# Fabri000/Maze-Solving-Agent-Gymnasium

Hardware: NVIDIA B200
Metric: env-steps/sec (40x40 mazes, whole job) (higher is better)
Workload: dtype u8/int32 state+obs, f64 reward

## Files before the change

### maze-solving-agent-gymnasium_b200/csrc/maze_abi.cu

```cuda
#include <cmath>
#include <cstdio>
#include <cstdlib>
#include <cstring>
#include <new>
#include "maze_common.cuh"

int maze_fail_cuda(maze_ctx* ctx, cudaError_t e, const char* what) {
    if (ctx) snprintf(ctx->err, sizeof(ctx->err), "CUDA error %d (%s) in %s", (int)e, cudaGetErrorString(e), what);
    return (int)e;
}

int maze_fail_arg(maze_ctx* ctx, int code, const char* what) {
    if (ctx) snprintf(ctx->err, sizeof(ctx->err), "argument error %d: %s", code, what);
    return code;
}

int maze_check_batch(maze_ctx* ctx, const maze_env_batch* b) {
    if (!b) return maze_fail_arg(ctx, MAZE_E_NULL, "batch");
    if (!b->meta || !b->table || !b->env_maze || !b->state || !b->visits || !b->agent || !b->target ||
        !b->best_dir || !b->reward || !b->terminated || !b->truncated)
        return maze_fail_arg(ctx, MAZE_E_NULL, "batch pointer");
    if (b->num_envs <= 0 || b->num_mazes <= 0 || b->slot <= 0 || (b->slot & 1))
        return maze_fail_arg(ctx, MAZE_E_RANGE, "num_envs / num_mazes / slot (must be even)");
    if (b->visit_slot < b->slot || (b->visit_tiled != 0 && b->visit_tiled != 1))
        return maze_fail_arg(ctx, MAZE_E_RANGE, "visit_slot (>= slot) / visit_tiled (0 or 1)");
    if (b->visit_bits && (b->visit_bits_pitch < 1 || b->visit_bits_stride < b->visit_bits_pitch || (b->visit_bits_stride & 3) ||
                          ((uintptr_t)b->visit_bits & 15)))
        return maze_fail_arg(ctx, MAZE_E_RANGE, "visit_bits: pitch >= 1, stride a multiple of 4 words, 16-byte aligned");
    if (b->visit_cell_stride <= 0 || b->visit_env_stride <= 0)
        return maze_fail_arg(ctx, MAZE_E_RANGE, "visit strides (cell-major: B, 1; env-major: 1, slot)");
    if (((uintptr_t)b->meta & 15) || ((uintptr_t)b->state & 7) || ((uintptr_t)b->agent & 7) ||
        ((uintptr_t)b->target & 7) || ((uintptr_t)b->best_dir & 7) || ((uintptr_t)b->reward & 7) ||
        ((uintptr_t)b->visits & 3))
        return maze_fail_arg(ctx, MAZE_E_ALIGN, "batch pointer alignment");
    return 0;
}


extern "C" int maze_abi_version(void) { return MAZE_ABI_VERSION; }

extern "C" int maze_sizeof(int which) {
    switch (which) {
        case 0: return (int)sizeof(maze_env_batch);
        case 1: return (int)sizeof(maze_q_agent);
        case 2: return (int)sizeof(maze_replay);
        case 3: return (int)sizeof(maze_step_trace);
        case 4: return (int)sizeof(maze_dqn_net);
        default: return -1;
    }
}

extern "C" int maze_ctx_create(maze_ctx** out, int device) {
    if (!out) return MAZE_E_NULL;
    *out = nullptr;
    maze_ctx* ctx = new (std::nothrow) maze_ctx();
    if (!ctx) return MAZE_E_RANGE;
    memset(ctx, 0, sizeof(*ctx));
    ctx->device = device;
    for (int i = 0; i < 256; ++i) {
        ctx->h_lut_revisit[i] = 0.0 - (1 - std::exp(-0.2 * i));
        ctx->h_lut_invalid[i] = 0.0 - (1 - std::exp(-0.15 * i));
    }
    ctx->h_shaping[0] = 0 * 0.5 - 0.05;
    ctx->h_shaping[1] = 1 * 0.5 - 0.05;
    ctx->h_shaping[2] = 0.0;
    ctx->h_shaping[3] = -1 * 0.5 - 0.05;
    cudaError_t e = cudaSetDevice(device);
    if (e == cudaSuccess) e = cudaMalloc(&ctx->d_lut_revisit, 256 * sizeof(double));
    if (e == cudaSuccess) e = cudaMalloc(&ctx->d_lut_invalid, 256 * sizeof(double));
    if (e == cudaSuccess) e = cudaMalloc(&ctx->d_counter, 4 * sizeof(int));
    if (e == cudaSuccess) e = cudaMemcpy(ctx->d_lut_revisit, ctx->h_lut_revisit, 256 * sizeof(double), cudaMemcpyHostToDevice);
    if (e == cudaSuccess) e = cudaMemcpy(ctx->d_lut_invalid, ctx->h_lut_invalid, 256 * sizeof(double), cudaMemcpyHostToDevice);
    if (e == cudaSuccess) e = cudaDeviceGetAttribute(&ctx->num_sms, cudaDevAttrMultiProcessorCount, device);
    if (e != cudaSuccess) {
        int rc = (int)e;
        cudaFree(ctx->d_lut_revisit);
        cudaFree(ctx->d_lut_invalid);
        cudaFree(ctx->d_counter);
        delete ctx;
        return rc;
    }
    ctx->step_ept = 2;
    if (const char* v = getenv("MAZE_STEP_EPT")) ctx->step_ept = atoi(v);
    if (const char* v = getenv("MAZE_L2_PERSIST_MB")) {
        int maxp = 0;
        cudaDeviceGetAttribute(&maxp, cudaDevAttrMaxPersistingL2CacheSize, device);
        size_t want = (size_t)atoi(v) << 20, before = 0, after = 0;
        if (want > (size_t)maxp) want = (size_t)maxp;
        cudaDeviceGetLimit(&before, cudaLimitPersistingL2CacheSize);
        cudaError_t le = cudaDeviceSetLimit(cudaLimitPersistingL2CacheSize, want);
        cudaDeviceGetLimit(&after, cudaLimitPersistingL2CacheSize);
        fprintf(stderr, "[maze_b200] persisting L2 %zu -> %zu bytes (max %d, rc %d)\n", before, after, maxp, (int)le);
    }
    if (const char* v = getenv("MAZE_L2_FETCH")) {
        size_t before = 0, after = 0;
        cudaDeviceGetLimit(&before, cudaLimitMaxL2FetchGranularity);
        cudaError_t le = cudaDeviceSetLimit(cudaLimitMaxL2FetchGranularity, (size_t)atoi(v));
        cudaDeviceGetLimit(&after, cudaLimitMaxL2FetchGranularity);
        fprintf(stderr, "[maze_b200] L2 fetch granularity %zu -> %zu (rc %d)\n", before, after, (int)le);
    }
    *out = ctx;
    return 0;
}

extern "C" void maze_ctx_destroy(maze_ctx* ctx) {
    if (!ctx) return;
    cudaFree(ctx->d_lut_revisit);
    cudaFree(ctx->d_lut_invalid);
    cudaFree(ctx->d_counter);
    cudaFree(ctx->d_scratch);
    maze_net_profile_free(ctx);
    delete ctx;
}

extern "C" const char* maze_last_error(maze_ctx* ctx) { return ctx ? ctx->err : "null ctx"; }

extern "C" int maze_reward_lut(maze_ctx* ctx, int kind, double* out) {
    if (!out) return MAZE_E_NULL;
    double rev[256], inv[256];
    for (int i = 0; i < 256; ++i) {
        rev[i] = 0.0 - (1 - std::exp(-0.2 * i));
        inv[i] = 0.0 - (1 - std::exp(-0.15 * i));
    }
    memset(out, 0, 256 * sizeof(double));
    if (kind == 0) memcpy(out, rev, sizeof(rev));
    else if (kind == 1) memcpy(out, inv, sizeof(inv));
    else if (kind == 2) { out[0] = -1 * 0.5 - 0.05; out[1] = 0 * 0.5 - 0.05; out[2] = 1 * 0.5 - 0.05; }
    else return maze_fail_arg(ctx, MAZE_E_RANGE, "maze_reward_lut kind");
    return 0;
}

extern "C" int maze_step_decode_host(const uint32_t* records, int64_t n, const int32_t* shape, const uint8_t* toroidal, int32_t* agent,
                                     int32_t* best_dir, double* reward, uint8_t* terminated, uint8_t* truncated) {
    if (!records || n < 0) return MAZE_E_NULL;
    double lut[4][256];
    memset(lut, 0, sizeof(lut));
    for (int i = 0; i < 256; ++i) {
        lut[MAZE_REC_KIND_REVISIT][i] = 0.0 - (1 - std::exp(-0.2 * i));
        lut[MAZE_REC_KIND_INVALID][i] = 0.0 - (1 - std::exp(-0.15 * i));
    }
    lut[MAZE_REC_KIND_SHAPING][0] = -1 * 0.5 - 0.05;
    lut[MAZE_REC_KIND_SHAPING][1] = 0 * 0.5 - 0.05;
    lut[MAZE_REC_KIND_SHAPING][2] = 1 * 0.5 - 0.05;
    lut[MAZE_REC_KIND_CONST][MAZE_REC_CONST_ONE] = 1.0;
    lut[MAZE_REC_KIND_CONST][MAZE_REC_CONST_MINUS_ONE] = -1.0;
    for (int64_t e = 0; e < n; ++e) {
        const uint32_t rec = records[e];
        const int r = (int)(rec & 0xff), c = (int)((rec >> 8) & 0xff), code = (int)((rec >> MAZE_REC_CODE_SHIFT) & 7);
        if (agent) { agent[2 * e] = r; agent[2 * e + 1] = c; }
        if (best_dir) {
            int br = 0, bc = 0;
            if (code < 4) {
                const int dr = (code == 0) - (code == 1), dc = (code == 2) - (code == 3);
                int nr = r + dr, nc = c + dc;
                if (toroidal && toroidal[e] && shape) {
                    const int H = shape[2 * e], W = shape[2 * e + 1];
                    nr = nr < 0 ? H - 1 : (nr >= H ? 0 : nr);
                    nc = nc < 0 ? W - 1 : (nc >= W ? 0 : nc);
                }
                br = r - nr;
                bc = c - nc;
            }
            best_dir[2 * e] = br;
            best_dir[2 * e + 1] = bc;
        }
        if (reward) reward[e] = lut[(rec >> MAZE_REC_KIND_SHIFT) & 3][(rec >> MAZE_REC_INDEX_SHIFT) & 0xff];
        if (terminated) terminated[e] = (uint8_t)((rec >> MAZE_REC_TERM_SHIFT) & 1);
        if (truncated) truncated[e] = (uint8_t)((rec >> MAZE_REC_TRUNC_SHIFT) & 1);
    }
    return 0;
}
```

### maze-solving-agent-gymnasium_b200/csrc/maze_common.cuh

```cuda
#pragma once
#include <cuda_runtime.h>
#include <stdint.h>
#include "maze_b200.h"

#define MAZE_CHECK(call)                                                          \
    do {                                                                          \
        cudaError_t _e = (call);                                                  \
        if (_e != cudaSuccess) return maze_fail_cuda(ctx, _e, #call);             \
    } while (0)

struct maze_ctx {
    int device;
    double* d_lut_revisit;
    double* d_lut_invalid;
    int*    d_counter;
    double h_lut_revisit[256];
    double h_lut_invalid[256];
    double h_shaping[4];
    int    num_sms;
    int    step_ept;
    void*  d_scratch;
    size_t scratch_bytes;
    void*  net_profile;
    char   err[512];
};

void maze_net_profile_free(maze_ctx* ctx);
int maze_fail_cuda(maze_ctx* ctx, cudaError_t e, const char* what);
int maze_fail_arg(maze_ctx* ctx, int code, const char* what);
int maze_check_batch(maze_ctx* ctx, const maze_env_batch* b);

struct EnvState {
    int r, c, consec, flags, steps, epoch, tab;
};

__device__ __forceinline__ EnvState unpack_state(uint64_t s) {
    EnvState e;
    e.r = (int)(s & 0xff);
    e.c = (int)((s >> 8) & 0xff);
    e.consec = (int)((s >> 16) & 0xff);
    e.flags = (int)((s >> 24) & 0xff);
    e.steps = (int)((s >> 32) & 0xffff);
    e.epoch = (int)((s >> 48) & 0xff);
    e.tab = (int)((s >> 56) & 0xff);
    return e;
}

__device__ __forceinline__ uint64_t pack_state(const EnvState& e) {
    uint32_t lo = (uint32_t)e.r | ((uint32_t)e.c << 8) | ((uint32_t)e.consec << 16) | ((uint32_t)e.flags << 24);
    uint32_t hi = (uint32_t)e.steps | ((uint32_t)e.epoch << 16) | ((uint32_t)e.tab << 24);
    return (uint64_t)lo | ((uint64_t)hi << 32);
}

__device__ __forceinline__ void action_delta(int a, int& dr, int& dc) {
    dr = (a == 0) - (a == 1);
    dc = (a == 2) - (a == 3);
}

__device__ __forceinline__ int2 best_dir_from_code(int code, int r, int c, int H, int W, bool tor) {
    if (code >= 4) return make_int2(0, 0);
    int dr, dc;
    action_delta(code, dr, dc);
    int nr = r + dr, nc = c + dc;
    if (tor) {
        nr = nr < 0 ? H - 1 : (nr >= H ? 0 : nr);
        nc = nc < 0 ? W - 1 : (nc >= W ? 0 : nc);
    }
    return make_int2(r - nr, c - nc);
}

__device__ __forceinline__ void st_cs(int2* p, int2 v) { __stcs(p, v); }
__device__ __forceinline__ void st_cs(double* p, double v) { __stcs(p, v); }

struct Philox {
    uint32_t k0, k1;
    uint32_t c0, c1, c2, c3;
    uint32_t o0, o1, o2, o3;
    int have;

    __host__ __device__ void init(uint64_t seed, uint64_t seq, uint32_t sub = 0) {
        k0 = (uint32_t)seed;
        k1 = (uint32_t)(seed >> 32);
        c0 = 0; c1 = sub;
        c2 = (uint32_t)seq;
        c3 = (uint32_t)(seq >> 32);
        have = 0;
    }
    __host__ __device__ static inline void mulhilo(uint32_t a, uint32_t b, uint32_t& hi, uint32_t& lo) {
        uint64_t p = (uint64_t)a * b;
        hi = (uint32_t)(p >> 32);
        lo = (uint32_t)p;
    }
    __host__ __device__ void refill() {
        uint32_t x0 = c0, x1 = c1, x2 = c2, x3 = c3, a = k0, b = k1;
#pragma unroll
        for (int i = 0; i < 10; ++i) {
            uint32_t hi0, lo0, hi1, lo1;
            mulhilo(0xD2511F53u, x0, hi0, lo0);
            mulhilo(0xCD9E8D57u, x2, hi1, lo1);
            uint32_t y0 = hi1 ^ x1 ^ a, y1 = lo1, y2 = hi0 ^ x3 ^ b, y3 = lo0;
            x0 = y0; x1 = y1; x2 = y2; x3 = y3;
            a += 0x9E3779B9u; b += 0xBB67AE85u;
        }
        o0 = x0; o1 = x1; o2 = x2; o3 = x3;
        if (++c0 == 0) ++c1;
        have = 4;
    }
    __host__ __device__ uint32_t next() {
        if (have == 0) refill();
        const uint32_t v = o0;
        o0 = o1; o1 = o2; o2 = o3;
        --have;
        return v;
    }
    __host__ __device__ uint32_t below(uint32_t n) {
        return (uint32_t)(((uint64_t)next() * n) >> 32);
    }
};
```

### maze-solving-agent-gymnasium_b200/csrc/maze_step.cu

```cuda
#include "maze_env.cuh"

namespace {

constexpr int STEP_THREADS = 256;
#ifndef MAZE_STEP_MINB1
#define MAZE_STEP_MINB1 6
#endif
#ifndef MAZE_STEP_MINB4
#define MAZE_STEP_MINB4 2
#endif
#ifndef MAZE_STEP_MINB2
#define MAZE_STEP_MINB2 5
#endif

template <int EPT, bool kStats, bool kTiled>
__global__ void __launch_bounds__(STEP_THREADS, EPT == 2 ? MAZE_STEP_MINB2 : (EPT == 1 ? MAZE_STEP_MINB1 : MAZE_STEP_MINB4))
maze_step_kernel(maze_env_batch b, const uint8_t* __restrict__ actions, uint32_t mode, StepLuts luts) {
    const int base = blockIdx.x * (STEP_THREADS * EPT) + threadIdx.x;

    const uint64_t pol_state = l2_policy<MAZE_STATE_POLICY>(), pol_table = l2_policy<MAZE_TABLE_POLICY>();
    uint64_t raw[EPT];
    int m[EPT], a[EPT];
    bool valid[EPT];
#pragma unroll
    for (int k = 0; k < EPT; ++k) {
        const int e = base + k * STEP_THREADS;
        valid[k] = e < b.num_envs;
        const int ee = valid[k] ? e : b.num_envs - 1;
        raw[k] = pol_load<MAZE_STATE_POLICY>(reinterpret_cast<const unsigned long long*>(b.state) + ee, pol_state);
        m[k] = pol_load<MAZE_STATE_POLICY>(b.env_maze + ee, pol_state);
        a[k] = __ldcs(actions + ee) & 3;
    }

    bool do_reset[EPT];
    int hw[EPT], tor[EPT];
#pragma unroll
    for (int k = 0; k < EPT; ++k) {
        const int flags = (int)((raw[k] >> 24) & 0xff);
        do_reset[k] = valid[k] && (mode & MAZE_STEP_AUTORESET) && (flags & MAZE_ST_NEEDS_RESET);
        if (do_reset[k] && (mode & MAZE_STEP_WIN_NEXT) && (flags & MAZE_ST_WON)) {
            m[k] += b.pool_stride;
            if (m[k] >= b.num_mazes) m[k] -= b.num_mazes;
            pol_store<MAZE_STATE_POLICY>(b.env_maze + base + k * STEP_THREADS, m[k], pol_state);
        }
        const int2 shape = __ldg(reinterpret_cast<const int2*>(b.meta + (size_t)m[k] * MAZE_META_WORDS));
        hw[k] = shape.x | (shape.y << 16);
        tor[k] = __ldg(b.meta + (size_t)m[k] * MAZE_META_WORDS + MAZE_META_FLAGS) & MAZE_FLAG_TOROIDAL;
    }

    int npos[EPT], idx[EPT], vidx[EPT], tb[EPT];
    bool inb[EPT];
#pragma unroll
    for (int k = 0; k < EPT; ++k) {
        const int H = hw[k] & 0xffff, W = hw[k] >> 16;
        const int r = (int)(raw[k] & 0xff), c = (int)((raw[k] >> 8) & 0xff);
        int dr, dc;
        action_delta(a[k], dr, dc);
        int nr = r + dr, nc = c + dc;
        if (tor[k]) {
            nr = nr < 0 ? H - 1 : (nr >= H ? 0 : nr);
            nc = nc < 0 ? W - 1 : (nc >= W ? 0 : nc);
            inb[k] = true;
        } else {
            inb[k] = (nr > 0) & (nr < H - 1) & (nc > 0) & (nc < W - 1);
        }
        if (do_reset[k]) {
            const int start = __ldg(b.meta + (size_t)m[k] * MAZE_META_WORDS + MAZE_META_START);
            nr = start & 0xffff;
            nc = start >> 16;
            inb[k] = true;
        }
        if (!inb[k]) { nr = r; nc = c; }
        npos[k] = nr | (nc << 16);
        idx[k] = nr * W + nc;
        vidx[k] = kTiled ? ((((nr >> 2) * ((W + 3) >> 2) + (nc >> 2)) << 4) | ((nr & 3) << 2) | (nc & 3)) : idx[k];
#ifdef MAZE_EXP_NOTABLE
        tb[k] = 1 | ((idx[k] & 3) << 1) | ((idx[k] & 3) << 4);
#else
        tb[k] = pol_load_nc<MAZE_TABLE_POLICY>(b.table + (size_t)m[k] * b.slot + idx[k], pol_table);
#endif
    }

    const uint64_t pol = l2_policy<MAZE_VISIT_POLICY>();
    uint32_t vis[EPT];
    bool moved[EPT];
#pragma unroll
    for (int k = 0; k < EPT; ++k) {
        moved[k] = valid[k] && !do_reset[k] && inb[k] && (tb[k] & MAZE_TAB_OPEN);
        vis[k] = 0;
#ifndef MAZE_EXP_NOVISIT
        if (moved[k]) vis[k] = visit_load(VISIT_AT(b, base + k * STEP_THREADS, vidx[k]), pol);
#endif
    }

#pragma unroll
    for (int k = 0; k < EPT; ++k) {
        const int e = base + k * STEP_THREADS;
        const int H = hw[k] & 0xffff, W = hw[k] >> 16;
        const int goal = __ldg(b.meta + (size_t)m[k] * MAZE_META_WORDS + MAZE_META_GOAL);
        const int max_steps = __ldg(b.meta + (size_t)m[k] * MAZE_META_WORDS + MAZE_META_MAX_STEPS);
        double reward = 0.0;
        int term = 0, trunc = 0;
        uint32_t rcode = MAZE_REC_REWARD(MAZE_REC_KIND_CONST, MAZE_REC_CONST_ZERO);
        bool wrapped = false;
        EnvState st = unpack_state(raw[k]);

        if (do_reset[k]) {
            begin_episode(st, npos[k], tb[k], wrapped);
            visit_bits_clear(b, e);
        } else if (valid[k]) {
            if (moved[k]) {
                const int cnt = ((int)(vis[k] >> 8) == st.epoch) ? (int)(vis[k] & 0xff) : 0;
                if (cnt == 0) {
                    if (npos[k] == goal) {
                        reward = 1.0;
                        term = 1;
                        rcode = MAZE_REC_REWARD(MAZE_REC_KIND_CONST, MAZE_REC_CONST_ONE);
                    } else {
                        const int dd = ((st.tab >> MAZE_TAB_D4_SHIFT) - (tb[k] >> MAZE_TAB_D4_SHIFT)) & 3;
                        reward = dd == 1 ? luts.shaping_closer : (dd == 3 ? luts.shaping_farther : luts.shaping_same);
                        rcode = MAZE_REC_REWARD(MAZE_REC_KIND_SHAPING, dd == 1 ? 2u : (dd == 3 ? 0u : 1u));
                    }
                } else {
                    reward = __ldg(luts.revisit + cnt);
                    rcode = MAZE_REC_REWARD(MAZE_REC_KIND_REVISIT, (uint32_t)cnt);
                }
#ifndef MAZE_EXP_NOVISIT
                visit_store(VISIT_AT(b, e, vidx[k]), (unsigned)((st.epoch << 8) | (cnt < 255 ? cnt + 1 : 255)), pol);
                visit_bit_set(b, e, npos[k] & 0xffff, npos[k] >> 16);
#endif
                st.r = npos[k] & 0xffff;
                st.c = npos[k] >> 16;
                st.tab = tb[k];
                st.consec = 0;
                int nm = (st.flags >> MAZE_ST_NMOVES_SHIFT) & 3;
                nm = nm < 2 ? nm + 1 : 2;
                st.flags = (a[k] << MAZE_ST_MOVE_SHIFT) | (nm << MAZE_ST_NMOVES_SHIFT);
            } else {
                st.consec = st.consec < 255 ? st.consec + 1 : 255;
                reward = __ldg(luts.invalid + st.consec);
                rcode = MAZE_REC_REWARD(MAZE_REC_KIND_INVALID, (uint32_t)st.consec);
                st.flags &= ~(MAZE_ST_NEEDS_RESET | MAZE_ST_WON);
            }
            st.steps = st.steps < 65535 ? st.steps + 1 : 65535;
            if (st.steps > max_steps) {
                trunc = 1;
                reward = -1.0;
                rcode = MAZE_REC_REWARD(MAZE_REC_KIND_CONST, MAZE_REC_CONST_MINUS_ONE);
            }
            if (term | trunc) st.flags |= MAZE_ST_NEEDS_RESET | (term ? MAZE_ST_WON : 0);
        }

        const unsigned need = __ballot_sync(0xffffffffu, wrapped);
        if (need) warp_clear_visits(need, b, e);
        if (kStats && b.stats) {
            const unsigned stepped = __ballot_sync(0xffffffffu, valid[k] && !do_reset[k]);
            if (stepped && (threadIdx.x & 31) == 0) atomicAdd(reinterpret_cast<unsigned long long*>(b.stats + 3), (unsigned long long)__popc(stepped));
        }

        if (!valid[k]) continue;

        pol_store<MAZE_STATE_POLICY>(reinterpret_cast<unsigned long long*>(b.state) + e, (unsigned long long)pack_state(st), pol_state);
        if (do_reset[k] && (raw[k] >> 24 & MAZE_ST_WON)) {
            st_cs(reinterpret_cast<int2*>(b.target) + e, make_int2(goal & 0xffff, goal >> 16));
            if (b.target_dirty) *b.target_dirty = 1;
        }
        if (mode & MAZE_STEP_PACKED)
            __stcs(b.packed + e, (uint32_t)st.r | ((uint32_t)st.c << 8) | ((uint32_t)((st.tab >> MAZE_TAB_CODE_SHIFT) & 7) << MAZE_REC_CODE_SHIFT) |
                                     ((uint32_t)term << MAZE_REC_TERM_SHIFT) | ((uint32_t)trunc << MAZE_REC_TRUNC_SHIFT) | rcode);
        if (!(mode & MAZE_STEP_NO_WIDE)) {
            st_cs(reinterpret_cast<int2*>(b.agent) + e, make_int2(st.r, st.c));
            st_cs(reinterpret_cast<int2*>(b.best_dir) + e,
                  best_dir_from_code((st.tab >> MAZE_TAB_CODE_SHIFT) & 7, st.r, st.c, H, W, tor[k] != 0));
            st_cs(b.reward + e, reward);
            __stcs(b.terminated + e, (uint8_t)term);
            __stcs(b.truncated + e, (uint8_t)trunc);
        }

        if (kStats) {
            if (b.ep_return) {
                double g = do_reset[k] ? 0.0 : b.ep_return[e] + reward;
                b.ep_return[e] = g;
                if ((term | trunc) && b.stats_return) atomicAdd(b.stats_return, g);
            }
            if (b.stats) {
                if (term | trunc) {
                    atomicAdd(reinterpret_cast<unsigned long long*>(b.stats + 0), 1ull);
                    if (term) atomicAdd(reinterpret_cast<unsigned long long*>(b.stats + 1), 1ull);
                    else atomicAdd(reinterpret_cast<unsigned long long*>(b.stats + 2), 1ull);
                }
            }
            if (term && (mode & MAZE_STEP_WIN_QUEUE) && b.queue) {
                int at = atomicAdd(b.queue_count, 1);
                b.queue[at] = m[k];
            }
        }
    }
}

__global__ void __launch_bounds__(STEP_THREADS)
maze_reset_kernel(maze_env_batch b, const uint8_t* __restrict__ mask) {
    const int e = blockIdx.x * STEP_THREADS + threadIdx.x;
    const bool valid = e < b.num_envs;
    const int ee = valid ? e : b.num_envs - 1;
    const bool sel = valid && (mask == nullptr || mask[ee] != 0);
    bool wrapped = false;
    EnvState s;
    int H = 0, W = 0, goal = 0;
    bool tor = false;
    if (sel) {
        s = unpack_state(b.state[ee]);
        const int m = b.env_maze[ee];
        const int4* mp = reinterpret_cast<const int4*>(b.meta + (size_t)m * MAZE_META_WORDS);
        const int4 m0 = __ldg(mp);
        const int4 m1 = __ldg(mp + 1);
        H = m0.x; W = m0.y; goal = m0.w;
        tor = (m1.y & MAZE_FLAG_TOROIDAL) != 0;
        const int start = m0.z;
        const int sidx = (start & 0xffff) * W + (start >> 16);
        begin_episode(s, start, __ldg(b.table + (size_t)m * b.slot + sidx), wrapped);
        visit_bits_clear(b, ee);
    }
    const unsigned need = __ballot_sync(0xffffffffu, wrapped);
    if (need) warp_clear_visits(need, b, ee);
    if (!sel) return;
    b.state[e] = pack_state(s);
    reinterpret_cast<int2*>(b.agent)[e] = make_int2(s.r, s.c);
    reinterpret_cast<int2*>(b.target)[e] = make_int2(goal & 0xffff, goal >> 16);
    if (b.target_dirty) *b.target_dirty = 1;
    reinterpret_cast<int2*>(b.best_dir)[e] =
        best_dir_from_code((s.tab >> MAZE_TAB_CODE_SHIFT) & 7, s.r, s.c, H, W, tor);
    b.reward[e] = 0.0;
    b.terminated[e] = 0;
    b.truncated[e] = 0;
    if (b.ep_return) b.ep_return[e] = 0.0;
}

__global__ void __launch_bounds__(STEP_THREADS)
maze_step_many_kernel(maze_env_batch b, const uint8_t* __restrict__ actions, int k_steps, uint32_t mode, StepLuts luts,
                      maze_step_trace tr, int e0, int e1) {
    const int e = e0 + blockIdx.x * STEP_THREADS + threadIdx.x;
    if (e >= e1) return;
    const size_t B = (size_t)b.num_envs;
    EnvState st = unpack_state(b.state[e]);
    int m = b.env_maze[e];
    MazeView mz = load_maze(b, m);
    double reward = 0.0, ep_return = b.ep_return ? b.ep_return[e] : 0.0;
    int term = 0, trunc = 0;
    bool target_changed = false;
    unsigned long long n_episodes = 0, n_wins = 0, n_steps = 0;
    double return_sum = 0.0;
    for (int k = 0; k < k_steps; ++k) {
        if ((mode & MAZE_STEP_AUTORESET) && (st.flags & MAZE_ST_NEEDS_RESET)) {
            if ((mode & MAZE_STEP_WIN_NEXT) && (st.flags & MAZE_ST_WON)) {
                m += b.pool_stride;
                if (m >= b.num_mazes) m -= b.num_mazes;
                mz = load_maze(b, m);
            }
            bool wrapped;
            begin_episode(st, mz.start, __ldg(mz.tab + (mz.start & 0xffff) * mz.W + (mz.start >> 16)), wrapped);
            visit_bits_clear(b, e);
            if (wrapped)
                for (int i = 0; i < b.visit_slot; ++i) *VISIT_AT(b, e, i) = 0;
            reward = 0.0; term = 0; trunc = 0;
            ep_return = 0.0;
            target_changed = true;
        } else {
            const StepResult r = env_transition(b, e, st, mz, __ldcs(actions + (size_t)k * B + e) & 3, luts);
            reward = r.reward; term = r.term; trunc = r.trunc;
            ep_return += reward;
            ++n_steps;
            if (term | trunc) {
                ++n_episodes;
                n_wins += term;
                return_sum += ep_return;
            }
        }
        const size_t at = (size_t)k * B + e;
        if (tr.agent) __stcs(reinterpret_cast<int2*>(tr.agent) + at, make_int2(st.r, st.c));
        if (tr.best_dir)
            __stcs(reinterpret_cast<int2*>(tr.best_dir) + at,
                   best_dir_from_code((st.tab >> MAZE_TAB_CODE_SHIFT) & 7, st.r, st.c, mz.H, mz.W, mz.tor));
        if (tr.reward) __stcs(tr.reward + at, reward);
        if (tr.terminated) __stcs(tr.terminated + at, (uint8_t)term);
        if (tr.truncated) __stcs(tr.truncated + at, (uint8_t)trunc);
    }
    b.state[e] = pack_state(st);
    b.env_maze[e] = m;
    reinterpret_cast<int2*>(b.agent)[e] = make_int2(st.r, st.c);
    if (target_changed) {
        reinterpret_cast<int2*>(b.target)[e] = make_int2(mz.goal & 0xffff, mz.goal >> 16);
        if (b.target_dirty) *b.target_dirty = 1;
    }
    reinterpret_cast<int2*>(b.best_dir)[e] = best_dir_from_code((st.tab >> MAZE_TAB_CODE_SHIFT) & 7, st.r, st.c, mz.H, mz.W, mz.tor);
    b.reward[e] = reward;
    b.terminated[e] = (uint8_t)term;
    b.truncated[e] = (uint8_t)trunc;
    if (b.ep_return) b.ep_return[e] = ep_return;
    if (b.stats && n_steps) atomicAdd(reinterpret_cast<unsigned long long*>(b.stats + 3), n_steps);
    if (n_episodes) {
        if (b.stats) {
            atomicAdd(reinterpret_cast<unsigned long long*>(b.stats + 0), n_episodes);
            if (n_wins) atomicAdd(reinterpret_cast<unsigned long long*>(b.stats + 1), n_wins);
            if (n_episodes - n_wins) atomicAdd(reinterpret_cast<unsigned long long*>(b.stats + 2), n_episodes - n_wins);
        }
        if (b.ep_return && b.stats_return) atomicAdd(b.stats_return, return_sum);
    }
}

}

extern "C" int maze_step_many(maze_ctx* ctx, const maze_env_batch* b, const uint8_t* actions, int k_steps, uint32_t mode,
                              const maze_step_trace* trace, int chunk_envs, void* stream) {
    if (!ctx) return MAZE_E_NULL;
    if (int rc = maze_check_batch(ctx, b)) return rc;
    if (!actions) return maze_fail_arg(ctx, MAZE_E_NULL, "maze_step_many: actions");
    if (k_steps < 1 || chunk_envs < 0) return maze_fail_arg(ctx, MAZE_E_RANGE, "maze_step_many: k_steps / chunk_envs");
    if (mode & MAZE_STEP_WIN_QUEUE)
        return maze_fail_arg(ctx, MAZE_E_RANGE, "maze_step_many: MAZE_STEP_WIN_QUEUE needs a generation launch between steps; use maze_step");
    maze_step_trace tr = {nullptr, nullptr, nullptr, nullptr, nullptr};
    if (trace) tr = *trace;
    if (((uintptr_t)tr.agent & 7) || ((uintptr_t)tr.best_dir & 7) || ((uintptr_t)tr.reward & 7))
        return maze_fail_arg(ctx, MAZE_E_ALIGN, "maze_step_many: trace pointer alignment");
    const int chunk = chunk_envs > 0 ? chunk_envs : b->num_envs;
    const StepLuts luts = step_luts(ctx);
    cudaStream_t st = static_cast<cudaStream_t>(stream);
    for (int e0 = 0; e0 < b->num_envs; e0 += chunk) {
        const int e1 = e0 + chunk < b->num_envs ? e0 + chunk : b->num_envs;
        maze_step_many_kernel<<<(e1 - e0 + STEP_THREADS - 1) / STEP_THREADS, STEP_THREADS, 0, st>>>(*b, actions, k_steps, mode, luts, tr, e0, e1);
    }
    MAZE_CHECK(cudaGetLastError());
    return 0;
}

extern "C" int maze_step(maze_ctx* ctx, const maze_env_batch* b, const uint8_t* actions, uint32_t mode, void* stream) {
    if (!ctx) return MAZE_E_NULL;
    if (int rc = maze_check_batch(ctx, b)) return rc;
    if (!actions) return maze_fail_arg(ctx, MAZE_E_NULL, "actions");
    if ((mode & MAZE_STEP_PACKED) && (!b->packed || ((uintptr_t)b->packed & 3)))
        return maze_fail_arg(ctx, MAZE_E_NULL, "maze_step: MAZE_STEP_PACKED needs batch.packed ([B] uint32)");
    if ((mode & MAZE_STEP_NO_WIDE) && !(mode & MAZE_STEP_PACKED))
        return maze_fail_arg(ctx, MAZE_E_RANGE, "maze_step: MAZE_STEP_NO_WIDE without MAZE_STEP_PACKED would drop the step's outputs");
    const StepLuts luts = step_luts(ctx);
    const bool stats = b->ep_return || b->stats || ((mode & MAZE_STEP_WIN_QUEUE) && b->queue);
    cudaStream_t st = static_cast<cudaStream_t>(stream);
    int ept = ctx->step_ept;
    if (b->num_envs < 64 * 1024) ept = 1;
    auto grid_for = [&](int e) { return (b->num_envs + STEP_THREADS * e - 1) / (STEP_THREADS * e); };
    auto launch = [&](auto kernel, int e) { kernel<<<grid_for(e), STEP_THREADS, 0, st>>>(*b, actions, mode, luts); };
#define MAZE_STEP_DISPATCH(EPT_)                                                                          \
    do {                                                                                                  \
        if (stats) { if (tiled) launch(maze_step_kernel<EPT_, true, true>, EPT_); else launch(maze_step_kernel<EPT_, true, false>, EPT_); } \
        else       { if (tiled) launch(maze_step_kernel<EPT_, false, true>, EPT_); else launch(maze_step_kernel<EPT_, false, false>, EPT_); } \
    } while (0)
    const bool tiled = b->visit_tiled != 0;
    if (ept >= 4) MAZE_STEP_DISPATCH(4);
    else if (ept == 2) MAZE_STEP_DISPATCH(2);
    else MAZE_STEP_DISPATCH(1);
#undef MAZE_STEP_DISPATCH
    MAZE_CHECK(cudaGetLastError());
    return 0;
}

extern "C" int maze_reset(maze_ctx* ctx, const maze_env_batch* b, const uint8_t* mask, void* stream) {
    if (!ctx) return MAZE_E_NULL;
    if (int rc = maze_check_batch(ctx, b)) return rc;
    const int grid = (b->num_envs + STEP_THREADS - 1) / STEP_THREADS;
    maze_reset_kernel<<<grid, STEP_THREADS, 0, static_cast<cudaStream_t>(stream)>>>(*b, mask);
    MAZE_CHECK(cudaGetLastError());
    return 0;
}
```

Baseline: 44.14 billion.

## Add specialized lean step kernel with mode templating and unified reward LUT

Adds a lean step kernel, templated on the step mode, for the common case: no stats, no visit bitmaps, untiled visits, and full CTAs. It reads rewards from a single combined device LUT indexed by record kind, uses a warp-uniform fast path for bordered mazes that skips toroidal wrapping and the general best-direction computation, and drops the tail guards. Any remaining envs fall back to the generic kernel, which now takes an offset. The aim is fewer branches and less per-thread work, at the cost of extra template instantiations, a possible second launch for the tail, and a MAZE_EXP_PAD experiment hook.

```diff
diff --git a/maze-solving-agent-gymnasium_b200/csrc/maze_abi.cu b/maze-solving-agent-gymnasium_b200/csrc/maze_abi.cu
--- a/maze-solving-agent-gymnasium_b200/csrc/maze_abi.cu
+++ b/maze-solving-agent-gymnasium_b200/csrc/maze_abi.cu
@@ -65,10 +65,21 @@
     ctx->h_shaping[1] = 1 * 0.5 - 0.05;
     ctx->h_shaping[2] = 0.0;
     ctx->h_shaping[3] = -1 * 0.5 - 0.05;
+    double lut_reward[4][256];
+    memset(lut_reward, 0, sizeof(lut_reward));
+    memcpy(lut_reward[MAZE_REC_KIND_REVISIT], ctx->h_lut_revisit, sizeof(ctx->h_lut_revisit));
+    memcpy(lut_reward[MAZE_REC_KIND_INVALID], ctx->h_lut_invalid, sizeof(ctx->h_lut_invalid));
+    lut_reward[MAZE_REC_KIND_SHAPING][0] = ctx->h_shaping[3];
+    lut_reward[MAZE_REC_KIND_SHAPING][1] = ctx->h_shaping[0];
+    lut_reward[MAZE_REC_KIND_SHAPING][2] = ctx->h_shaping[1];
+    lut_reward[MAZE_REC_KIND_CONST][MAZE_REC_CONST_ONE] = 1.0;
+    lut_reward[MAZE_REC_KIND_CONST][MAZE_REC_CONST_MINUS_ONE] = -1.0;
     cudaError_t e = cudaSetDevice(device);
     if (e == cudaSuccess) e = cudaMalloc(&ctx->d_lut_revisit, 256 * sizeof(double));
     if (e == cudaSuccess) e = cudaMalloc(&ctx->d_lut_invalid, 256 * sizeof(double));
+    if (e == cudaSuccess) e = cudaMalloc(&ctx->d_lut_reward, sizeof(lut_reward));
     if (e == cudaSuccess) e = cudaMalloc(&ctx->d_counter, 4 * sizeof(int));
+    if (e == cudaSuccess) e = cudaMemcpy(ctx->d_lut_reward, lut_reward, sizeof(lut_reward), cudaMemcpyHostToDevice);
     if (e == cudaSuccess) e = cudaMemcpy(ctx->d_lut_revisit, ctx->h_lut_revisit, 256 * sizeof(double), cudaMemcpyHostToDevice);
     if (e == cudaSuccess) e = cudaMemcpy(ctx->d_lut_invalid, ctx->h_lut_invalid, 256 * sizeof(double), cudaMemcpyHostToDevice);
     if (e == cudaSuccess) e = cudaDeviceGetAttribute(&ctx->num_sms, cudaDevAttrMultiProcessorCount, device);
@@ -76,12 +87,14 @@
         int rc = (int)e;
         cudaFree(ctx->d_lut_revisit);
         cudaFree(ctx->d_lut_invalid);
+        cudaFree(ctx->d_lut_reward);
         cudaFree(ctx->d_counter);
         delete ctx;
         return rc;
     }
     ctx->step_ept = 2;
     if (const char* v = getenv("MAZE_STEP_EPT")) ctx->step_ept = atoi(v);
+    if (const char* v = getenv("MAZE_STEP_GENERIC")) ctx->step_generic = atoi(v) != 0;
     if (const char* v = getenv("MAZE_L2_PERSIST_MB")) {
         int maxp = 0;
         cudaDeviceGetAttribute(&maxp, cudaDevAttrMaxPersistingL2CacheSize, device);
@@ -107,6 +120,7 @@
     if (!ctx) return;
     cudaFree(ctx->d_lut_revisit);
     cudaFree(ctx->d_lut_invalid);
+    cudaFree(ctx->d_lut_reward);
     cudaFree(ctx->d_counter);
     cudaFree(ctx->d_scratch);
     maze_net_profile_free(ctx);
diff --git a/maze-solving-agent-gymnasium_b200/csrc/maze_common.cuh b/maze-solving-agent-gymnasium_b200/csrc/maze_common.cuh
--- a/maze-solving-agent-gymnasium_b200/csrc/maze_common.cuh
+++ b/maze-solving-agent-gymnasium_b200/csrc/maze_common.cuh
@@ -17,8 +17,10 @@
     double h_lut_revisit[256];
     double h_lut_invalid[256];
     double h_shaping[4];
+    double* d_lut_reward;
     int    num_sms;
     int    step_ept;
+    int    step_generic;
     void*  d_scratch;
     size_t scratch_bytes;
     void*  net_profile;
@@ -69,6 +71,12 @@
     return make_int2(r - nr, c - nc);
 }
 
+__device__ __forceinline__ int2 best_dir_bordered(int code) {
+    int dr, dc;
+    action_delta(code, dr, dc);
+    return make_int2(-dr, -dc);
+}
+
 __device__ __forceinline__ void st_cs(int2* p, int2 v) { __stcs(p, v); }
 __device__ __forceinline__ void st_cs(double* p, double v) { __stcs(p, v); }
 
diff --git a/maze-solving-agent-gymnasium_b200/csrc/maze_step.cu b/maze-solving-agent-gymnasium_b200/csrc/maze_step.cu
--- a/maze-solving-agent-gymnasium_b200/csrc/maze_step.cu
+++ b/maze-solving-agent-gymnasium_b200/csrc/maze_step.cu
@@ -13,10 +13,24 @@
 #define MAZE_STEP_MINB2 5
 #endif
 
+__device__ __forceinline__ int exp_pad(uint64_t raw) {
+#ifdef MAZE_EXP_PAD
+    const uint32_t zero = (uint32_t)(raw >> 63);
+    uint32_t z = (uint32_t)raw;
+#pragma unroll
+    for (int i = 0; i < MAZE_EXP_PAD / 2; ++i) asm volatile("add.u32 %0, %0, %1;\n\txor.b32 %0, %0, %1;" : "+r"(z) : "r"(zero));
+    return (int)(z - (uint32_t)raw);
+#else
+    (void)raw;
+    return 0;
+#endif
+}
+
+#define MAZE_STEP_MINB(EPT) (EPT == 2 ? MAZE_STEP_MINB2 : (EPT == 1 ? MAZE_STEP_MINB1 : MAZE_STEP_MINB4))
 template <int EPT, bool kStats, bool kTiled>
-__global__ void __launch_bounds__(STEP_THREADS, EPT == 2 ? MAZE_STEP_MINB2 : (EPT == 1 ? MAZE_STEP_MINB1 : MAZE_STEP_MINB4))
-maze_step_kernel(maze_env_batch b, const uint8_t* __restrict__ actions, uint32_t mode, StepLuts luts) {
-    const int base = blockIdx.x * (STEP_THREADS * EPT) + threadIdx.x;
+__global__ void __launch_bounds__(STEP_THREADS, MAZE_STEP_MINB(EPT))
+maze_step_kernel(maze_env_batch b, const uint8_t* __restrict__ actions, uint32_t mode, StepLuts luts, int e0) {
+    const int base = e0 + blockIdx.x * (STEP_THREADS * EPT) + threadIdx.x;
 
     const uint64_t pol_state = l2_policy<MAZE_STATE_POLICY>(), pol_table = l2_policy<MAZE_TABLE_POLICY>();
     uint64_t raw[EPT];
@@ -150,6 +164,7 @@
             }
             if (term | trunc) st.flags |= MAZE_ST_NEEDS_RESET | (term ? MAZE_ST_WON : 0);
         }
+        st.steps += exp_pad(raw[k]);
 
         const unsigned need = __ballot_sync(0xffffffffu, wrapped);
         if (need) warp_clear_visits(need, b, e);
@@ -195,6 +210,164 @@
                 b.queue[at] = m[k];
             }
         }
+    }
+}
+
+template <int EPT, uint32_t kMode>
+__global__ void __launch_bounds__(STEP_THREADS, MAZE_STEP_MINB(EPT))
+maze_step_lean_kernel(maze_env_batch b, const uint8_t* __restrict__ actions, const double* __restrict__ rewards) {
+    constexpr bool kAutoreset = (kMode & MAZE_STEP_AUTORESET) != 0, kWinNext = (kMode & MAZE_STEP_WIN_NEXT) != 0;
+    constexpr bool kPacked = (kMode & MAZE_STEP_PACKED) != 0, kWide = (kMode & MAZE_STEP_NO_WIDE) == 0;
+    const int base = blockIdx.x * (STEP_THREADS * EPT) + threadIdx.x;
+
+    const uint64_t pol_state = l2_policy<MAZE_STATE_POLICY>(), pol_table = l2_policy<MAZE_TABLE_POLICY>();
+    uint64_t raw[EPT];
+    int m[EPT], a[EPT];
+#pragma unroll
+    for (int k = 0; k < EPT; ++k) {
+        const int e = base + k * STEP_THREADS;
+        raw[k] = pol_load<MAZE_STATE_POLICY>(reinterpret_cast<const unsigned long long*>(b.state) + e, pol_state);
+        m[k] = pol_load<MAZE_STATE_POLICY>(b.env_maze + e, pol_state);
+        a[k] = __ldcs(actions + e) & 3;
+    }
+
+    bool do_reset[EPT], tor[EPT];
+    int4 rec[EPT];
+    int max_steps[EPT];
+    bool any_tor = false;
+#pragma unroll
+    for (int k = 0; k < EPT; ++k) {
+        const int flags = (int)((raw[k] >> 24) & 0xff);
+        do_reset[k] = kAutoreset && (flags & MAZE_ST_NEEDS_RESET);
+        if (kWinNext && do_reset[k] && (flags & MAZE_ST_WON)) {
+            m[k] += b.pool_stride;
+            if (m[k] >= b.num_mazes) m[k] -= b.num_mazes;
+            pol_store<MAZE_STATE_POLICY>(b.env_maze + base + k * STEP_THREADS, m[k], pol_state);
+        }
+        const int4* mp = reinterpret_cast<const int4*>(b.meta) + 2u * (uint32_t)m[k];
+        rec[k] = __ldg(mp);
+        const int4 r1 = __ldg(mp + 1);
+        max_steps[k] = r1.x;
+        tor[k] = (r1.y & MAZE_FLAG_TOROIDAL) != 0;
+        any_tor |= tor[k];
+    }
+    const bool bordered = !__any_sync(0xffffffffu, any_tor);
+
+    int npos[EPT], idx[EPT], tb[EPT];
+    bool inb[EPT];
+#pragma unroll
+    for (int k = 0; k < EPT; ++k) {
+        const int H = rec[k].x, W = rec[k].y;
+        const int r = (int)(raw[k] & 0xff), c = (int)((raw[k] >> 8) & 0xff);
+        int dr, dc;
+        action_delta(a[k], dr, dc);
+        int nr = r + dr, nc = c + dc;
+        if (!bordered && tor[k]) {
+            nr = nr < 0 ? H - 1 : (nr >= H ? 0 : nr);
+            nc = nc < 0 ? W - 1 : (nc >= W ? 0 : nc);
+            inb[k] = true;
+        } else {
+            inb[k] = (nr > 0) & (nr < H - 1) & (nc > 0) & (nc < W - 1);
+        }
+        if (do_reset[k]) {
+            nr = rec[k].z & 0xffff;
+            nc = rec[k].z >> 16;
+            inb[k] = true;
+        }
+        if (!inb[k]) { nr = r; nc = c; }
+        npos[k] = nr | (nc << 16);
+        idx[k] = nr * W + nc;
+        tb[k] = pol_load_nc<MAZE_TABLE_POLICY>(b.table + ((uint32_t)m[k] * (uint32_t)b.slot + (uint32_t)idx[k]), pol_table);
+    }
+
+    const uint64_t pol = l2_policy<MAZE_VISIT_POLICY>();
+    uint16_t* vp[EPT];
+    uint32_t vis[EPT];
+    bool moved[EPT];
+#pragma unroll
+    for (int k = 0; k < EPT; ++k) {
+        moved[k] = !do_reset[k] && inb[k] && (tb[k] & MAZE_TAB_OPEN);
+        vp[k] = VISIT_AT(b, base + k * STEP_THREADS, idx[k]);
+        vis[k] = 0;
+#ifndef MAZE_EXP_NOVISIT
+        if (moved[k]) vis[k] = visit_load(vp[k], pol);
+#endif
+    }
+
+#pragma unroll
+    for (int k = 0; k < EPT; ++k) {
+        const int e = base + k * STEP_THREADS;
+        const int goal = rec[k].w;
+        int ri = MAZE_REC_KIND_CONST * 256 + MAZE_REC_CONST_ZERO;
+        int term = 0, trunc = 0;
+        bool wrapped = false;
+        EnvState st = unpack_state(raw[k]);
+
+        if (do_reset[k]) {
+            begin_episode(st, npos[k], tb[k], wrapped);
+        } else {
+            if (moved[k]) {
+                const int cnt = ((int)(vis[k] >> 8) == st.epoch) ? (int)(vis[k] & 0xff) : 0;
+                const int dd = ((st.tab >> MAZE_TAB_D4_SHIFT) - (tb[k] >> MAZE_TAB_D4_SHIFT)) & 3;
+                term = cnt == 0 && npos[k] == goal;
+                ri = cnt ? MAZE_REC_KIND_REVISIT * 256 + cnt
+                         : (term ? MAZE_REC_KIND_CONST * 256 + MAZE_REC_CONST_ONE : MAZE_REC_KIND_SHAPING * 256 + ((0x19 >> (2 * dd)) & 3));
+#ifndef MAZE_EXP_NOVISIT
+                visit_store(vp[k], (unsigned)((st.epoch << 8) | (cnt < 255 ? cnt + 1 : 255)), pol);
+#endif
+                st.r = npos[k] & 0xffff;
+                st.c = npos[k] >> 16;
+                st.tab = tb[k];
+                st.consec = 0;
+                int nm = (st.flags >> MAZE_ST_NMOVES_SHIFT) & 3;
+                nm = nm < 2 ? nm + 1 : 2;
+                st.flags = (a[k] << MAZE_ST_MOVE_SHIFT) | (nm << MAZE_ST_NMOVES_SHIFT);
+            } else {
+                st.consec = st.consec < 255 ? st.consec + 1 : 255;
+                ri = MAZE_REC_KIND_INVALID * 256 + st.consec;
+                st.flags &= ~(MAZE_ST_NEEDS_RESET | MAZE_ST_WON);
+            }
+            st.steps = st.steps < 65535 ? st.steps + 1 : 65535;
+            if (st.steps > max_steps[k]) {
+                trunc = 1;
+                ri = MAZE_REC_KIND_CONST * 256 + MAZE_REC_CONST_MINUS_ONE;
+            }
+            if (term | trunc) st.flags |= MAZE_ST_NEEDS_RESET | (term ? MAZE_ST_WON : 0);
+        }
+        st.steps += exp_pad(raw[k]);
+
+        const unsigned need = __ballot_sync(0xffffffffu, wrapped);
+        if (need) warp_clear_visits(need, b, e);
+
+        pol_store<MAZE_STATE_POLICY>(reinterpret_cast<unsigned long long*>(b.state) + e, (unsigned long long)pack_state(st), pol_state);
+        if (do_reset[k] && (raw[k] >> 24 & MAZE_ST_WON)) {
+            st_cs(reinterpret_cast<int2*>(b.target) + e, make_int2(goal & 0xffff, goal >> 16));
+            if (b.target_dirty) *b.target_dirty = 1;
+        }
+        const int code = (st.tab >> MAZE_TAB_CODE_SHIFT) & 7;
+        if (kPacked)
+            __stcs(b.packed + e, (uint32_t)st.r | ((uint32_t)st.c << 8) | ((uint32_t)code << MAZE_REC_CODE_SHIFT) | ((uint32_t)term << MAZE_REC_TERM_SHIFT) |
+                                     ((uint32_t)trunc << MAZE_REC_TRUNC_SHIFT) | MAZE_REC_REWARD(ri >> 8, ri & 0xff));
+        if (kWide) {
+            st_cs(reinterpret_cast<int2*>(b.agent) + e, make_int2(st.r, st.c));
+            st_cs(reinterpret_cast<int2*>(b.best_dir) + e,
+                  bordered ? best_dir_bordered(code) : best_dir_from_code(code, st.r, st.c, rec[k].x, rec[k].y, tor[k]));
+            st_cs(b.reward + e, __ldg(rewards + ri));
+            __stcs(b.terminated + e, (uint8_t)term);
+            __stcs(b.truncated + e, (uint8_t)trunc);
+        }
+    }
+}
+
+template <int EPT>
+bool launch_lean(uint32_t mode, int grid, const maze_env_batch& b, const uint8_t* actions, const double* rewards, cudaStream_t s) {
+    constexpr uint32_t AR = MAZE_STEP_AUTORESET, WN = MAZE_STEP_WIN_NEXT, PK = MAZE_STEP_PACKED, NW = MAZE_STEP_NO_WIDE;
+    switch (mode) {
+        case AR | WN:           maze_step_lean_kernel<EPT, AR | WN><<<grid, STEP_THREADS, 0, s>>>(b, actions, rewards); return true;
+        case AR | WN | PK:      maze_step_lean_kernel<EPT, AR | WN | PK><<<grid, STEP_THREADS, 0, s>>>(b, actions, rewards); return true;
+        case AR | WN | PK | NW: maze_step_lean_kernel<EPT, AR | WN | PK | NW><<<grid, STEP_THREADS, 0, s>>>(b, actions, rewards); return true;
+        case AR:                maze_step_lean_kernel<EPT, AR><<<grid, STEP_THREADS, 0, s>>>(b, actions, rewards); return true;
+        default:                return false;
     }
 }
 
@@ -343,21 +516,34 @@
         return maze_fail_arg(ctx, MAZE_E_RANGE, "maze_step: MAZE_STEP_NO_WIDE without MAZE_STEP_PACKED would drop the step's outputs");
     const StepLuts luts = step_luts(ctx);
     const bool stats = b->ep_return || b->stats || ((mode & MAZE_STEP_WIN_QUEUE) && b->queue);
+    const bool tiled = b->visit_tiled != 0;
     cudaStream_t st = static_cast<cudaStream_t>(stream);
-    int ept = ctx->step_ept;
+    int ept = ctx->step_ept >= 4 ? 4 : (ctx->step_ept == 2 ? 2 : 1);
     if (b->num_envs < 64 * 1024) ept = 1;
-    auto grid_for = [&](int e) { return (b->num_envs + STEP_THREADS * e - 1) / (STEP_THREADS * e); };
-    auto launch = [&](auto kernel, int e) { kernel<<<grid_for(e), STEP_THREADS, 0, st>>>(*b, actions, mode, luts); };
-#define MAZE_STEP_DISPATCH(EPT_)                                                                          \
-    do {                                                                                                  \
-        if (stats) { if (tiled) launch(maze_step_kernel<EPT_, true, true>, EPT_); else launch(maze_step_kernel<EPT_, true, false>, EPT_); } \
-        else       { if (tiled) launch(maze_step_kernel<EPT_, false, true>, EPT_); else launch(maze_step_kernel<EPT_, false, false>, EPT_); } \
-    } while (0)
-    const bool tiled = b->visit_tiled != 0;
-    if (ept >= 4) MAZE_STEP_DISPATCH(4);
-    else if (ept == 2) MAZE_STEP_DISPATCH(2);
-    else MAZE_STEP_DISPATCH(1);
+    const int per_cta = STEP_THREADS * ept;
+    int e0 = 0;
+    if (!ctx->step_generic && !stats && !b->visit_bits && !tiled && (uint64_t)b->num_mazes * (uint64_t)b->slot < (1ull << 32) &&
+        b->num_envs >= per_cta) {
+        const uint32_t lean_mode = mode & ~MAZE_STEP_WIN_QUEUE;
+        const int grid = b->num_envs / per_cta;
+        const bool ok = ept == 4 ? launch_lean<4>(lean_mode, grid, *b, actions, ctx->d_lut_reward, st)
+                      : ept == 2 ? launch_lean<2>(lean_mode, grid, *b, actions, ctx->d_lut_reward, st)
+                                 : launch_lean<1>(lean_mode, grid, *b, actions, ctx->d_lut_reward, st);
+        if (ok) e0 = grid * per_cta;
+    }
+    if (e0 < b->num_envs) {
+        const int grid = (b->num_envs - e0 + per_cta - 1) / per_cta;
+        auto launch = [&](auto kernel) { kernel<<<grid, STEP_THREADS, 0, st>>>(*b, actions, mode, luts, e0); };
+#define MAZE_STEP_DISPATCH(EPT_)                                                                                           \
+        do {                                                                                                               \
+            if (stats) { if (tiled) launch(maze_step_kernel<EPT_, true, true>); else launch(maze_step_kernel<EPT_, true, false>); }   \
+            else       { if (tiled) launch(maze_step_kernel<EPT_, false, true>); else launch(maze_step_kernel<EPT_, false, false>); } \
+        } while (0)
+        if (ept == 4) MAZE_STEP_DISPATCH(4);
+        else if (ept == 2) MAZE_STEP_DISPATCH(2);
+        else MAZE_STEP_DISPATCH(1);
 #undef MAZE_STEP_DISPATCH
+    }
     MAZE_CHECK(cudaGetLastError());
     return 0;
 }
```

Measured after the change: 44.79 billion (median of 6 runs). 1.5% higher.
